# ZYM-PKU/UDiffText

Hardware: AMD Instinct MI355X
Metric: 512x512 50-step denoised images/sec (UDiffText hot path: conditioner + 50 CFG Euler steps + VAE decode) (higher is better)
Workload: dtype bf16; 1 GPU; 512x512, 50 Euler/DDIM(eta 0) steps, CFG 5.0, 9-char labels, noise_iters 0; global batch 4 per step sharded over 1 GPU(s) = 4 images per GPU in micro-batches of 4: every UNet call runs ONE batch of 4 (8 samples with CFG); 3 such batch(es) in flight per GPU on separate launch streams; BASELINE.json configs[1]; global_batch=4, weights=synthetic (name-keyed recipe), 1361.2 M parameters, launch=hipGraph replay of the sampler steps, in_flight=3, batches_per_unet_call=1

## Files before the change

udifftext_amd/csrc/gemm.hip:

```cpp
#include "common.h"
#include <stdio.h>
#include <stdlib.h>
#include <string.h>
#include <atomic>
#include <cmath>

hipError_t udt_lean_launch_gemm(int cfg, const void* lparams, int smem, int G, int geglu, int ln, hipStream_t s);
hipError_t udt_lean_launch_conv3(const void* c3params, hipStream_t s);

namespace {
#include "tile_common.h"

struct GemmParams {
  const uint16_t* a;
  const uint16_t* a2;
  const uint16_t* w;
  const uint16_t* zero;
  const float* bias;
  const uint16_t* res;
  const float* rowvec;
  void* out;
  const float* colscale;
  const float* in_scsh;
  float* colstats;
// ... 821 lines not shown
  t.G = round_workgroups(units);
  int nb = g_n_block.load(std::memory_order_relaxed);
  if (nb <= 0) nb = (t.tiles_m <= 8) ? t.tiles_n : 8;
  if (nb > t.tiles_n) nb = t.tiles_n;
  t.n_block = nb;
  return true;
}

size_t lean_workspace(const LeanPlan& t) {
  return t.splitk > 1 ? G8_HEADER_BYTES + (size_t)t.tiles * t.splitk * t.bm * t.bn * sizeof(float) : 0;
}

std::atomic<int> g_lean_conv{-1};
std::atomic<int> g_wide_conv{-2};
int wide_conv_mode() {
  int v = g_wide_conv.load(std::memory_order_relaxed);
  if (v == -2) {
    const char* e = getenv("UDT_WIDE_CONV");
    v = e ? atoi(e) : -1;
    g_wide_conv.store(v, std::memory_order_relaxed);
  }
  return v;
}
#ifdef UDT_MEASURE
std::atomic<int> g_lconv_dbg{0};
#endif

std::atomic<int> g_wide_lanes_eff{-2};
double wide_lanes_eff() {
  int v = g_wide_lanes_eff.load(std::memory_order_relaxed);
  if (v == -2) {
    const char* e = getenv("UDT_WIDE_LANES_EFF");
    v = e ? atoi(e) : 70;
    g_wide_lanes_eff.store(v, std::memory_order_relaxed);
  }
  return v / 100.0;
}

int conv_chunk_slices(long long tiles, int slots, int chunks, int knob) {
  long long sk = 1;
  if (tiles <= 1023) {
    if (knob > 1) { sk = knob; if (sk > chunks) sk = chunks; }
    else if (knob < 0 && tiles * 2 <= slots && chunks >= 10) { sk = slots / tiles; if (sk > chunks / 4) sk = chunks / 4; }
    if (sk < 1) sk = 1;
  }
  return (int)sk;
}

bool lean_conv_plan(const udt_gemm_desc* d, lg::C3Params& c, bool want_stats) {
  int on = g_lean_conv.load(std::memory_order_relaxed);
  if (on < 0) {
    const char* e = getenv("UDT_LEAN_CONV");
    on = (e && e[0] == '0') ? 0 : 1;
    g_lean_conv.store(on, std::memory_order_relaxed);
  }
  if (!on || lean_mode() == 0) return false;
  if (d->flags != UDT_GEMM_CONV || d->ksize != 3 || d->stride != 1 || d->pad_t != 1 || d->pad_l != 1) return false;
  if (d->C2 != 0 || d->in_scsh || d->colscale || d->batch > 1) return false;
  if (want_stats && !lean_stats_enabled()) return false;
  if (d->N < 128 || d->N % 8 != 0 || d->C1 <= 0 || d->C1 % 64 != 0) return false;
  if (d->upsample != 0 && d->upsample != 1 && d->upsample != 2) return false;
  const bool phase = d->upsample == 2, ups = d->upsample == 1;
  const int nph = phase ? 4 : 1;
  if (d->Hout != (d->Hin << (d->upsample ? 1 : 0)) || d->Wout != (d->Win << (d->upsample ? 1 : 0))) return false;
  if (phase && d->ldw > 0 && d->ldw < 4 * d->C1) return false;
  const int Ht = phase ? d->Hin : d->Hout, Wt = phase ? d->Win : d->Wout;
  c.bn = 128; c.wgm = 2;
  bool wide = false;
  int wide_slots = device_cus();
  {
    const int wm = wide_conv_mode();
    if (wm != 0 && !ups && d->N % 160 == 0 && Wt % 16 == 0 && Ht % 16 == 0) {
      const int cus = device_cus(), share = d->cu_share > 1 ? d->cu_share : 1;
      wide_slots = cus / share > 0 ? cus / share : 1;
      const long long wt = (long long)(d->M / 256) * (d->N / 160);
      const long long sk = conv_chunk_slices(wt, wide_slots, d->C1 / 64, lean_splitk_knob());
      const long long units = wt * sk;
      const long long rounds = (units + cus - 1) / cus;
      const double eff = units > cus ? (double)units / (double)(rounds * cus) : ((double)units * share >= cus ? 1.0 : (double)units * share / cus);
      wide = (wm > 0) || (sk <= 2 && eff >= ((share >= 3 && share_of(d) >= 3) ? wide_lanes_eff() : 0.85));
    }
  }
  if (wide) { c.geo = phase ? 6 : 3; c.tw = 16; c.th = 16; c.bn = 160; c.wgm = 4; }
  else if (Wt % 16 == 0 && Ht % 8 == 0) { c.geo = ups ? 2 : phase ? 4 : 0; c.tw = 16; c.th = 8; }
  else if (!ups && Wt % 8 == 0 && Ht % 8 == 0) { c.geo = phase ? 5 : 1; c.tw = 8; c.th = 8; }
  else return false;
  if (d->ldo % 8 != 0 || (d->residual && d->ldr % 8 != 0)) return false;
  const long long ldw = d->ldw > 0 ? d->ldw : (phase ? 4LL * d->C1 : (long long)d->K);
  if (ldw % 8 != 0) return false;
  c.w_phase = phase ? (d->stride_w > 0 ? d->stride_w : (long long)d->N * ldw) : 0;
  if (phase && (c.w_phase < (long long)d->N * ldw || c.w_phase % 8 != 0)) return false;
  if ((long long)d->M * d->C1 * 2 >= (1LL << 31) || (long long)d->N * ldw * 2 >= (1LL << 31)) return false;
  if ((reinterpret_cast<uintptr_t>(d->out) | reinterpret_cast<uintptr_t>(d->residual) | reinterpret_cast<uintptr_t>(d->bias) |
       reinterpret_cast<uintptr_t>(d->rowvec)) & 15) return false;
  if (d->rowvec && ((d->ld_rowvec > 0 ? d->ld_rowvec : d->N) % 4 != 0)) return false;
  c.dbg = 0;
#ifdef UDT_MEASURE
  c.dbg = g_lconv_dbg.load(std::memory_order_relaxed);
#endif
  c.N = d->N; c.C = d->C1; c.H = d->Hin; c.W = d->Win; c.B = d->M / (d->Hout * d->Wout);
  c.ldw = (int)ldw; c.ldo = d->ldo; c.ldr = d->ldr; c.ldrv = d->ld_rowvec > 0 ? d->ld_rowvec : d->N;
  c.alpha = d->alpha;
  c.tiles_x = Wt / c.tw; c.tiles_y = Ht / c.th;
  c.tiles_m = c.B * c.tiles_x * c.tiles_y;
  c.tiles_n = (d->N + c.bn - 1) / c.bn;
  c.tiles = c.tiles_m * c.tiles_n;
  c.chunks = c.C / 64;
  const int slots = wide ? wide_slots : (2 * device_cus() / share_of(d) > 0 ? 2 * device_cus() / share_of(d) : 1);
  int sk = conv_chunk_slices((long long)c.tiles * nph, slots, c.chunks, lean_splitk_knob());
  while (sk > 1 && (long long)c.tiles * nph * sk * c.tw * c.th * c.bn * 4 > (64LL << 20)) --sk;
  c.ch_per = (c.chunks + sk - 1) / sk;
  c.splitk = (c.chunks + c.ch_per - 1) / c.ch_per;
  c.G = round_workgroups(c.tiles * nph * c.splitk);
  {
    const double patch = (double)((ups ? c.tw / 2 : c.tw) + 2) * ((ups ? c.th / 2 : c.th) + 2) * c.C * 2.0, wtile = (phase ? 4.0 : 9.0) * c.bn * c.C * 2.0;
    int nb = g_n_block.load(std::memory_order_relaxed);
    if (nb <= 0) nb = (int)(std::sqrt(64.0 * patch / wtile) + 0.5);
    if (nb < 1) nb = 1;
    if (nb > c.tiles_n) nb = c.tiles_n;
    c.n_block = nb;
  }
  c.a_bytes = (unsigned)((long long)c.B * d->Hin * d->Win * d->C1 * 2);
  c.w_bytes = (unsigned)((long long)d->N * ldw * 2);
  c.counters = nullptr; c.slabs = nullptr;
  return true;
}

int lean_conv_phases(const lg::C3Params& c) { return c.geo >= 4 ? 4 : 1; }

size_t lean_conv_workspace(const lg::C3Params& c) {
  return c.splitk > 1 ? G8_HEADER_BYTES + (size_t)c.tiles * lean_conv_phases(c) * c.splitk * c.tw * c.th * c.bn * sizeof(float) : 0;
}

bool lean_stats_probe(const udt_gemm_desc* d, int& rows, int& slots) {
  if (d->in_scsh) return false;
  {
    lg::C3Params c3;
    if (lean_conv_plan(d, c3, true)) {
      rows = c3.tw * c3.th / c3.wgm;
      slots = c3.tiles_m * c3.wgm * lean_conv_phases(c3);
      return true;
    }
  }
  if ((d->flags & UDT_GEMM_CONV) && d->ksize == 3) return false;
  LeanPlan lt;
  if (lean_plan(d, lt, true)) {
    rows = lt.stats_rows;
    slots = lt.tiles_m * (lt.bm / lt.stats_rows);
    return true;
  }
  return false;
}
}

extern "C" int udt_debug_set(const char* key, int32_t value) {
  if (!key) return UDT_ERR_BAD_ARG;
  if (!strcmp(key, "n_block")) { g_n_block.store(value); return UDT_OK; }
  if (!strcmp(key, "rows_epi")) { g_rows_epi.store(value ? 1 : 0); return UDT_OK; }
  if (!strcmp(key, "lean")) { g_lean.store(value < 0 ? -2 : value); return UDT_OK; }
  if (!strcmp(key, "rowres")) { g_rowres.store(value < 0 ? 1 : (value ? 1 : 0)); return UDT_OK; }
  if (!strcmp(key, "wide_lanes_eff")) { g_wide_lanes_eff.store(value < 0 ? -2 : value); return UDT_OK; }
  if (!strcmp(key, "conv_n4")) { g_conv_n4.store(value < 0 ? -2 : (value ? 1 : 0)); return UDT_OK; }
  if (!strcmp(key, "lean256_lanes")) { g_lean256_lanes.store(value < 0 ? -2 : (value ? 1 : 0)); return UDT_OK; }
  if (!strcmp(key, "lean_splitk")) { g_lean_splitk.store(value); return UDT_OK; }
  if (!strcmp(key, "share_splitk")) { g_share_splitk.store(value < 0 ? -2 : (value ? 1 : 0)); return UDT_OK; }
  if (!strcmp(key, "lean_conv")) { g_lean_conv.store(value < 0 ? -1 : (value ? 1 : 0)); return UDT_OK; }
  if (!strcmp(key, "wide_conv")) { g_wide_conv.store(value < 0 ? -1 : (value ? 1 : 0)); return UDT_OK; }
#ifdef UDT_MEASURE
  if (!strcmp(key, "lconv_dbg")) { g_lconv_dbg.store(value); return UDT_OK; }
  static const struct { const char* k; int bit; } bits[] = {{"no_xchg", 28}, {"no_epi", 27}, {"no_store", 26}, {"no_res", 25},
                                                            {"no_bias", 24}, {"no_fast", 22}};
  for (const auto& b : bits)
    if (!strcmp(key, b.k)) {
      int cur = g_dbg_bits.load();
      g_dbg_bits.store((cur & ~(1 << b.bit)) | (value ? (1 << b.bit) : 0));
      return UDT_OK;
    }
#endif
  return UDT_ERR_BAD_ARG;
}

extern "C" int udt_check_async_error(void* workspace, size_t workspace_bytes, void* stream) {
  if (!workspace || workspace_bytes < G8_HEADER_BYTES) return UDT_ERR_BAD_ARG;
  hipStream_t s = reinterpret_cast<hipStream_t>(stream);
  int err = 0;
  hipError_t e = hipMemcpyAsync(&err, reinterpret_cast<int*>(workspace) + 1023, sizeof(int), hipMemcpyDeviceToHost, s);
  if (e == hipSuccess) e = hipStreamSynchronize(s);
  if (e != hipSuccess) return udt_set_hip_error(e);
  if (err == 0) return UDT_OK;
  e = hipMemsetAsync(workspace, 0, G8_HEADER_BYTES, s);
// ... 7 lines not shown
extern "C" int32_t udt_gemm_q8_ok(const udt_gemm_desc* d) {
  if (!d || !d->q8_out || d->M <= 0 || d->N <= 0 || d->K <= 0) return 0;
  LeanPlan lt;
  return lean_plan(d, lt, d->colstats != nullptr) ? 1 : 0;
}

extern "C" int32_t udt_gemm_rowstat_parts(const udt_gemm_desc* d) {
  if (!d || d->M <= 0 || d->N <= 0 || d->K <= 0) return 0;
  udt_gemm_desc t = *d;
  alignas(16) static const uint64_t probe_dst[2] = {0, 0};
  if (!t.q8_out) { t.q8_out = const_cast<uint64_t*>(probe_dst); t.q8_scale = const_cast<uint64_t*>(probe_dst); if (t.ld_q8 <= 0) t.ld_q8 = (t.N + 15) / 16 * 16; }
  LeanPlan lt;
  if (!lean_plan(&t, lt, false) || lt.cfg != 1 || (d->flags & UDT_GEMM_GEGLU)) return 0;
  return (d->N + 63) / 64;
}
extern "C" int32_t udt_gemm_in_scsh_ok(const udt_gemm_desc* d) {
  if (!d || d->K <= 0 || d->K % BK != 0) return 0;
  c3p::Geo ge;
  return conv3p_geometry(d, ge, true) ? 1 : 0;
}

extern "C" int32_t udt_gemm_up4_ok(const udt_gemm_desc* d) {
  if (!d || d->upsample != 2) return 0;
  lg::C3Params c3;
  return lean_conv_plan(d, c3, d->colstats != nullptr) ? 1 : 0;
}

extern "C" int udt_gn_silu_conv3x3_fwd(const udt_gemm_desc* d, void* workspace, size_t workspace_bytes, void* stream) {
  if (!d || !(d->flags & UDT_GEMM_CONV) || d->ksize != 3 || d->stride != 1 || d->pad_t != 1 || d->pad_l != 1 || !d->in_scsh)
    return UDT_ERR_BAD_ARG;
  return udt_gemm(d, workspace, workspace_bytes, stream);
}

extern "C" int udt_ln_gemm_fwd(const udt_gemm_desc* d, void* workspace, size_t workspace_bytes, void* stream) {
  if (!d || !d->ln_colsum || !d->bias || !(d->ln_eps > 0.f)) return UDT_ERR_BAD_ARG;
  LeanPlan lt;
  if (!lean_plan(d, lt, false)) return UDT_ERR_BAD_SHAPE;
  return udt_gemm(d, workspace, workspace_bytes, stream);
}

extern "C" size_t udt_gemm_workspace_bytes(const udt_gemm_desc* d) {
  if (!d || d->K <= 0 || d->M <= 0 || d->N <= 0 || d->K % k_tile(d) != 0) return 0;
  if (conv_n4_applies(d)) return 0;
  {
    LeanPlan lt;
    if (lean_plan(d, lt, d->colstats != nullptr)) return lean_workspace(lt);
// ... 162 lines not shown
        udt_prof_tag(profl.rec, tag);
      }
      const bool geglu = (d->flags & UDT_GEMM_GEGLU) != 0, ln = d->ln_colsum != nullptr;
      hipError_t el;
      el = udt_lean_launch_gemm(lt.cfg, &lp, lt.smem, lt.G, geglu ? 1 : 0, ln ? 1 : 0, s);
      if (el != hipSuccess) return udt_set_hip_error(el);
      return UDT_OK;
    }
  }
  if (d->ln_colsum) return UDT_ERR_BAD_ARG;
  {
    lg::C3Params c3;
    if (lean_conv_plan(d, c3, d->colstats != nullptr)) {
      c3.colstats = d->colstats;
      c3.a = p.a; c3.w = p.w; c3.bias = p.bias; c3.res = p.res; c3.rowvec = p.rowvec; c3.out = reinterpret_cast<uint16_t*>(d->out);
      if (c3.splitk > 1) {
        if (!workspace || workspace_bytes < lean_conv_workspace(c3)) return UDT_ERR_WORKSPACE;
        c3.counters = reinterpret_cast<int*>(workspace);
        c3.slabs = reinterpret_cast<float*>(reinterpret_cast<char*>(workspace) + G8_HEADER_BYTES);
      }
      UdtProfScope profc(cls, s);
      if (profc.rec) {
        char tag[96];
        snprintf(tag, sizeof(tag), "%s%s M=%d N=%d K=%d %dx%d tile=%dx%d units=%d splitk=%d nb=%d%s", (c3.geo == 3 || c3.geo == 6) ? "wconv3" : "lconv3",
                 (d->upsample && c3.geo != 6) ? "+up" : "", d->M, d->N, d->K,
                 d->Hin, d->Win, c3.tw, c3.th, c3.tiles * lean_conv_phases(c3) * c3.splitk, c3.splitk, c3.n_block,
                 d->upsample == 2 ? " up4" : "");
        udt_prof_tag(profc.rec, tag);
      }
      const hipError_t ec = udt_lean_launch_conv3(&c3, s);
      if (ec != hipSuccess) return udt_set_hip_error(ec);
      return UDT_OK;
    }
  }
  {
    c3p::CParams cp;
    if (conv3p_geometry(d, cp.geo, d->in_scsh != nullptr)) {
      const TilePlan t3 = plan_tiles3p(d, cp.geo);
      p.tiles_m = t3.tiles_m; p.tiles_n = t3.tiles_n; p.tiles_per_batch = t3.tiles_m * t3.tiles_n;
      {
        const double patch = (double)cp.geo.prows_img * cp.geo.NI * cp.geo.C * 2.0;
        const double wtile = 9.0 * t3.bn * cp.geo.C * 2.0;
        const double S = (double)(t3.tiles < t3.G ? t3.tiles : t3.G) / 8.0;
        int nb = (int)(std::sqrt((S < 1.0 ? 1.0 : S) * patch / wtile) + 0.5);
        if (nb < 1) nb = 1;
        if (nb > t3.tiles_n) nb = t3.tiles_n;
        p.n_block = nb;
      }
      p.n_ktiles = t3.nkt;
      p.total_iters = t3.total;
// ... 110 lines not shown
```

udifftext_amd/csrc/lean.h:

```cpp
#pragma once

namespace lg {

using g8::wait_vm;
UDT_DEVINL void raw_barrier() {
  asm volatile("s_waitcnt lgkmcnt(0)" ::: "memory");
  __builtin_amdgcn_s_barrier();
  asm volatile("" ::: "memory");
}
using g8::buf_lds16;
using g8::OOB;

typedef __attribute__((ext_vector_type(2))) __bf16 bf2_t;
UDT_DEVINL float dot2_bf16(uint32_t a, uint32_t b, float c) {
  return __builtin_amdgcn_fdot2_f32_bf16(__builtin_bit_cast(bf2_t, a), __builtin_bit_cast(bf2_t, b), c, false);
}

template <int CPR, int RPI>
UDT_DEVINL void wave_colstats(char* wl, int lane, const float (&cs)[8], const float (&cq)[8], float* dst, bool col_ok) {
#pragma unroll
  for (int h = 0; h < 2; ++h) {
    f32x4 a = {cs[4 * h + 0], cs[4 * h + 1], cs[4 * h + 2], cs[4 * h + 3]};
    f32x4 b = {cq[4 * h + 0], cq[4 * h + 1], cq[4 * h + 2], cq[4 * h + 3]};
    *reinterpret_cast<f32x4*>(wl + lane * 64 + h * 16) = a;
// ... 563 lines not shown
              cs[2 * j + 1] += bb; cq[2 * j + 1] += bb * bb;
            }
          }
        }
      }
    }
    if constexpr (STATS) {
      const int slot = (m0 + row0) / WROWS;
      wave_colstats<CPR, RPI>(wl, lane, cs, cq, p.colstats + ((long long)slot * p.N + n) * 2, col_ok);
    }
  }
}


template <int MAXN>
UDT_DEVINL void wait_vm_upto(int n) {
  if constexpr (MAXN == 0) wait_vm<0>();
  else {
    if (n >= MAXN) wait_vm<MAXN>();
    else wait_vm_upto<MAXN - 1>(n);
  }
}

template <int TW, int TH, bool UPS>
struct C3Geo {
  static constexpr int PX = TW * TH;
  static constexpr int TM = PX / 64;
  static constexpr int PW = (UPS ? TW / 2 : TW) + 2, PH = (UPS ? TH / 2 : TH) + 2;
  static constexpr int PROWS = PW * PH;
  static constexpr int PIECES = (PROWS + 7) / 8;
  static constexpr int PATCH_BYTES = PIECES * 1024;
  static constexpr int W_BYTES = 128 * ROW_BYTES;
  static constexpr int NRING = (3 * W_BYTES + 2 * PATCH_BYTES <= 80 * 1024) ? 3 : 2;
  static constexpr int RING = NRING * W_BYTES + 2 * PATCH_BYTES;
  static constexpr int STAGING = 4 * TM * 32 * 256;
  static constexpr int SMEM = RING > STAGING ? RING : STAGING;
  static_assert(PX == 128 || PX == 64, "128 or 64 output pixels per workgroup");
  static_assert(SMEM <= 80 * 1024, "two workgroups per CU");
};

template <int TW, int TH, bool UPS, bool STATS = false, bool PHASE = false>
__global__ void __launch_bounds__(256, 2) lconv3_kernel(const C3Params p) {
  static_assert(!(UPS && PHASE), "the phase form runs on the low-resolution geometries");
  using Geo = C3Geo<TW, TH, UPS>;
  constexpr int NT = PHASE ? 4 : 9;
  constexpr int NW = 4, TM = Geo::TM, TN = 2, BN = 128, BMPX = Geo::PX;
  constexpr int C3_PW = Geo::PW, C3_PROWS = Geo::PROWS, C3_PIECES = Geo::PIECES, C3_PATCH_BYTES = Geo::PATCH_BYTES;
  constexpr int C3_W_BYTES = Geo::W_BYTES, C3_TW = TW, C3_TH = TH;
  constexpr int WROWS = TM * 32;
  constexpr int WP = 4;
  constexpr int PP = (C3_PIECES + NW - 1) / NW;
  constexpr int EROW = 64 * 4;
  extern __shared__ __attribute__((aligned(16))) char smem[];
  char* const wring = smem;
  constexpr int NR = Geo::NRING;
  char* const patches = smem + NR * C3_W_BYTES;

  const int tid = threadIdx.x;
  const int wave = __builtin_amdgcn_readfirstlane(tid >> 6);
  const int lane = tid & 63;
  const int l31 = lane & 31;
  const int hi = lane >> 5;
  const int l3 = lane >> 3;
  const int pslot = lane & 7;
  const int wm = wave >> 1, wn = wave & 1;
  const int row0 = wm * WROWS, col0 = wn * 64;
  const int swz_w = (l31 >> 1) & 7;
  const int w_frag_row = (col0 + l31) * ROW_BYTES;

  const int unit = range_index(blockIdx.x, p.G);
  if (unit >= p.tiles * p.splitk * (PHASE ? 4 : 1)) return;
  const int phase = PHASE ? unit / (p.tiles * p.splitk) : 0;
  const int pha = phase >> 1, phb = phase & 1;
  const int ptile = unit / p.splitk;
// ... 11 lines not shown
  }
  const int per_img = p.tiles_x * p.tiles_y;
  const int b = tile_m / per_img;
  const int rt = tile_m - b * per_img;
  const int ty = rt / p.tiles_x;
  const int y0 = ty * C3_TH, x0 = (rt - ty * p.tiles_x) * C3_TW;
  const int c0 = slice * p.ch_per;
  int c1 = c0 + p.ch_per;
  if (c1 > p.chunks) c1 = p.chunks;

  const __amdgpu_buffer_rsrc_t rsrc_a = __builtin_amdgcn_make_buffer_rsrc(const_cast<uint16_t*>(p.a), 0, p.a_bytes, 0x00020000);
  const __amdgpu_buffer_rsrc_t rsrc_w =
      __builtin_amdgcn_make_buffer_rsrc(const_cast<uint16_t*>(p.w) + (PHASE ? (long long)phase * p.w_phase : 0LL), 0, p.w_bytes, 0x00020000);
  auto patch_swz = [](int prow, int yy) { return ((prow - 2 * yy) >> 1) & 7; };
  unsigned w_voff[WP], p_voff[PP];
  int p_piece[PP];
#pragma unroll
  for (int i = 0; i < WP; ++i) {
    const int row = (wave + NW * i) * 8 + l3;
    const int kw = (pslot ^ ((row >> 1) & 7)) * 8;
    const int n = n0 + row;
    w_voff[i] = (n < p.N) ? (unsigned)(((long long)n * p.ldw + kw) * 2) : OOB;
  }
#pragma unroll
  for (int i = 0; i < PP; ++i) {
    int idx = wave + NW * i;
    while (idx >= C3_PIECES) idx -= NW;
    p_piece[i] = idx;
    const int prow = idx * 8 + l3;
    const int yy = prow / C3_PW;
    const int xx = prow - yy * C3_PW;
    const int gy = (UPS ? (y0 >> 1) : y0) + yy - 1, gx = (UPS ? (x0 >> 1) : x0) + xx - 1;
    const bool ok = (prow < C3_PROWS) && ((unsigned)gy < (unsigned)p.H) && ((unsigned)gx < (unsigned)p.W);
    const int koff = (pslot ^ patch_swz(prow, yy)) * 8;
    p_voff[i] = ok ? (unsigned)(((((long long)b * p.H + gy) * p.W + gx) * p.C + koff) * 2) : OOB;
  }
  int a_prow[TM], a_py[TM];
#pragma unroll
  for (int tm = 0; tm < TM; ++tm) {
    const int ml = row0 + tm * 32 + l31;
    const int py = ml / TW, px = ml - py * TW;
    a_py[tm] = PHASE ? py + pha : py;
    a_prow[tm] = UPS ? (py | (px << 16)) : PHASE ? ((py + pha) * C3_PW + px + phb) : (py * C3_PW + px);
  }
  auto issue_w = [&](int st, int c, int tap) {
    const int soff = (tap * p.C + c * 64) * 2;
    char* wbuf = wring + st * C3_W_BYTES;
#pragma unroll
    for (int i = 0; i < WP; ++i) buf_lds16(rsrc_w, wbuf + (wave + NW * i) * 1024, w_voff[i], soff);
  };
  auto issue_patch = [&](int c) {
    char* pbuf = patches + (c & 1) * C3_PATCH_BYTES;
#pragma unroll
    for (int i = 0; i < PP; ++i) buf_lds16(rsrc_a, pbuf + p_piece[i] * 1024, p_voff[i], c * 128);
  };

  f32x16 acc[TM][TN];
#pragma unroll
  for (int i = 0; i < TM; ++i)
#pragma unroll
    for (int j = 0; j < TN; ++j)
#pragma unroll
      for (int r = 0; r < 16; ++r) acc[i][j][r] = 0.f;

  issue_patch(c0);
#pragma unroll
  for (int j = 0; j < NR - 1; ++j) issue_w(j, c0, j);
  static_assert(NR - 1 < NT, "the ring's prologue stays inside the first chunk");
  int st = 0;
  for (int c = c0; c < c1; ++c) {
    const bool nxt = (c + 1 < c1);
    const char* pbuf = patches + (c & 1) * C3_PATCH_BYTES;
#pragma unroll
    for (int tap = 0; tap < NT; ++tap) {
      {
        const int w_ahead = nxt ? NR - 2 : ((NT - 1 - tap) < NR - 2 ? (NT - 1 - tap) : NR - 2);
        const bool patch_ahead = nxt && tap >= 1 && tap <= NR - 1;
        wait_vm_upto<(NR - 2) * WP + PP>(w_ahead * WP + (patch_ahead ? PP : 0));
      }
      raw_barrier();
      if (!UDT_DBG(p.dbg, 0)) {
        const int ahead = tap + NR - 1;
        int s2 = st + NR - 1;
        if (s2 >= NR) s2 -= NR;
        if (ahead < NT) issue_w(s2, c, ahead);
        else if (nxt) issue_w(s2, c + 1, ahead - NT);
      }
      if (tap == 0 && nxt && !UDT_DBG(p.dbg, 1)) issue_patch(c + 1);
      const int dy = PHASE ? tap >> 1 : tap / 3, dx = PHASE ? tap & 1 : tap - dy * 3;
      const char* wbuf = wring + st * C3_W_BYTES;
      bf16x8_t fx[4][TM], fw[4][TN];
      if (!UDT_DBG(p.dbg, 3)) {
#pragma unroll
        for (int t = 0; t < TM; ++t) {
          int prow, yy;
          if constexpr (UPS) {
            const int py = a_prow[t] & 0xffff, px = a_prow[t] >> 16;
            yy = ((py + dy - 1) >> 1) + 1;
            prow = yy * C3_PW + (((px + dx - 1) >> 1) + 1);
          } else {
            yy = a_py[t] + dy;
            prow = a_prow[t] + dy * C3_PW + dx;
          }
          const int arow = prow * ROW_BYTES, aswz = patch_swz(prow, yy);
#pragma unroll
          for (int ks = 0; ks < 4; ++ks) fx[ks][t] = lds_read_frag(pbuf + arow + (((ks * 2 + hi) ^ aswz) << 4));
        }
#pragma unroll
        for (int ks = 0; ks < 4; ++ks) {
          const int slot = ((ks * 2 + hi) ^ swz_w) << 4;
#pragma unroll
          for (int t = 0; t < TN; ++t) fw[ks][t] = lds_read_frag(wbuf + w_frag_row + t * 32 * ROW_BYTES + slot);
        }
      }
      if (UDT_DBG(p.dbg, 2)) {
#pragma unroll
        for (int ks = 0; ks < 4; ++ks) {
#pragma unroll
          for (int tm = 0; tm < TM; ++tm) asm volatile("" ::"v"(fx[ks][tm]));
#pragma unroll
          for (int tn = 0; tn < TN; ++tn) asm volatile("" ::"v"(fw[ks][tn]));
        }
      } else {
#pragma unroll
        for (int ks = 0; ks < 4; ++ks)
#pragma unroll
          for (int tm = 0; tm < TM; ++tm)
// ... 63 lines not shown
      for (int q = 0; q < 4; ++q) {
        const int chunk = (tn * 8 + q * 2 + hi) ^ (row & 7);
        f32x4 v = {acc[tm][tn][q * 4 + 0], acc[tm][tn][q * 4 + 1], acc[tm][tn][q * 4 + 2], acc[tm][tn][q * 4 + 3]};
        *reinterpret_cast<f32x4*>(wl + row * EROW + chunk * 16) = v;
      }
  }
  const int rl = lane >> 3, c8 = lane & 7;
  const int n = n0 + col0 + c8 * 8;
  const bool col_ok = n < p.N;
  f32x4 b0 = {0.f, 0.f, 0.f, 0.f}, b1 = b0;
  if (col_ok) {
    if (p.bias) {
      b0 = *reinterpret_cast<const f32x4*>(p.bias + n);
      b1 = *reinterpret_cast<const f32x4*>(p.bias + n + 4);
    }
    if (p.rowvec) {
      const float* rvp = p.rowvec + (long long)b * p.ldrv + n;
      const f32x4 r0 = *reinterpret_cast<const f32x4*>(rvp), r1 = *reinterpret_cast<const f32x4*>(rvp + 4);
#pragma unroll
      for (int j = 0; j < 4; ++j) b0[j] += r0[j], b1[j] += r1[j];
    }
  }
  constexpr int NIT = TM * 4;
  const int Ho = (UPS || PHASE) ? 2 * p.H : p.H, Wo = (UPS || PHASE) ? 2 * p.W : p.W;
  long long mrow[NIT];
#pragma unroll
  for (int i = 0; i < NIT; ++i) {
    const int ml = row0 + i * 8 + rl;
    const int py = ml / TW, px = ml - py * TW;
    mrow[i] = PHASE ? ((long long)b * Ho + (2 * (y0 + py) + pha)) * Wo + (2 * (x0 + px) + phb)
                    : ((long long)b * Ho + (y0 + py)) * Wo + (x0 + px);
  }
  u32x4 rv[NIT];
  if (p.res) {
#pragma unroll
    for (int i = 0; i < NIT; ++i) {
      u32x4 z = {0u, 0u, 0u, 0u};
      rv[i] = z;
      if (col_ok) rv[i] = *reinterpret_cast<const u32x4*>(p.res + mrow[i] * p.ldr + n);
    }
  }
  float cs[8], cq[8];
#pragma unroll
  for (int j = 0; j < 8; ++j) cs[j] = cq[j] = 0.f;
#pragma unroll
  for (int i = 0; i < NIT; ++i) {
    const int row = i * 8 + rl;
// ... 38 lines not shown
```

udifftext_amd/csrc/lean.hip:

```cpp
#include "common.h"
#include <stdio.h>
#include <stdlib.h>
#include <atomic>

namespace {
#include "tile_common.h"
#include "lean_params.h"
#include "lean.h"
#include "wide.h"
#include "rowres.h"

template <int NW, int WGM, int WGN, int TM, int TN, int NST, int TMB = TM>
hipError_t launch_lean(const lg::LParams& lp, int smem, int G, bool geglu, bool ln, hipStream_t s) {
  static AttrOnce once[5];
  const void* fn;
  const bool stats = lp.colstats != nullptr;
  if constexpr (NW == 4 && NST == 2) {
    if (stats) {
      fn = (const void*)lg::lgemm_kernel<NW, WGM, WGN, TM, TN, NST, false, false, TMB, true>;
      hipError_t e = once[4].ensure(fn, smem);
      if (e != hipSuccess) return e;
      void* args[] = {const_cast<lg::LParams*>(&lp)};
      return hipLaunchKernel(fn, dim3(G), dim3(NW * 64), args, smem, s);
    }
// ... 14 lines not shown
template <bool GEGLU, bool LN, bool STATS, bool FP8, bool EMIT>
hipError_t launch_lean_mx8_k(const lg::LParams& lp, int smem, int G, hipStream_t s) {
  static AttrOnce once;
  const void* fn = (const void*)lg::lgemm_kernel<4, 2, 2, 2, 2, 2, GEGLU, LN, 2, STATS, FP8, EMIT>;
  hipError_t e = once.ensure(fn, smem);
  if (e != hipSuccess) return e;
  void* args[] = {const_cast<lg::LParams*>(&lp)};
  return hipLaunchKernel(fn, dim3(G), dim3(256), args, smem, s);
}
hipError_t launch_lean_mx8(const lg::LParams& lp, int smem, int G, bool geglu, bool ln, bool fp8, bool emit, hipStream_t s) {
  const bool stats = lp.colstats != nullptr;
  if (!fp8) {
    if (emit && !geglu && !ln && !stats) return launch_lean_mx8_k<false, false, false, false, true>(lp, smem, G, s);
    return hipErrorInvalidValue;
  }
  if (geglu) return (ln && emit && !stats) ? launch_lean_mx8_k<true, true, false, true, true>(lp, smem, G, s) : hipErrorInvalidValue;
  if (ln) return stats ? hipErrorInvalidValue
                 : emit ? launch_lean_mx8_k<false, true, false, true, true>(lp, smem, G, s)
                        : launch_lean_mx8_k<false, true, false, true, false>(lp, smem, G, s);
  if (stats) return emit ? hipErrorInvalidValue : launch_lean_mx8_k<false, false, true, true, false>(lp, smem, G, s);
  return emit ? launch_lean_mx8_k<false, false, false, true, true>(lp, smem, G, s) : launch_lean_mx8_k<false, false, false, true, false>(lp, smem, G, s);
}

template <int TW, int TH, bool UPS, bool STATS, bool PHASE>
hipError_t launch_lconv3s(const lg::C3Params& c3, hipStream_t s) {
  static AttrOnce once;
  constexpr int smem = lg::C3Geo<TW, TH, UPS>::SMEM;
  hipError_t e = once.ensure(reinterpret_cast<const void*>(lg::lconv3_kernel<TW, TH, UPS, STATS, PHASE>), smem);
  if (e != hipSuccess) return e;
  hipLaunchKernelGGL((lg::lconv3_kernel<TW, TH, UPS, STATS, PHASE>), dim3(c3.G), dim3(256), smem, s, c3);
  return hipGetLastError();
}
template <int TW, int TH, bool UPS, bool PHASE = false>
hipError_t launch_lconv3(const lg::C3Params& c3, hipStream_t s) {
  return c3.colstats ? launch_lconv3s<TW, TH, UPS, true, PHASE>(c3, s) : launch_lconv3s<TW, TH, UPS, false, PHASE>(c3, s);
}

template <bool STATS, bool PHASE>
hipError_t launch_wconv3s(const lg::C3Params& c3, hipStream_t s) {
  static AttrOnce once;
  constexpr int smem = wd::WGeo::SMEM;
  hipError_t e = once.ensure(reinterpret_cast<const void*>(wd::wconv3_kernel<STATS, PHASE>), smem);
  if (e != hipSuccess) return e;
  hipLaunchKernelGGL((wd::wconv3_kernel<STATS, PHASE>), dim3(c3.G), dim3(256), smem, s, c3);
  return hipGetLastError();
}
template <int KT, bool GEGLU, bool EMIT = false>
hipError_t launch_rowres(const lg::LParams& lp, int G, hipStream_t s) {
  static AttrOnce once;
  constexpr int smem = rr::RGeo<KT, GEGLU>::SMEM;
  hipError_t e = once.ensure(reinterpret_cast<const void*>(rr::rgemm_kernel<KT, GEGLU, EMIT>), smem);
  if (e != hipSuccess) return e;
  hipLaunchKernelGGL((rr::rgemm_kernel<KT, GEGLU, EMIT>), dim3(G), dim3(256), smem, s, lp);
  return hipGetLastError();
}

template <bool PHASE>
hipError_t launch_wconv3(const lg::C3Params& c3, hipStream_t s) {
// ... 2 lines not shown

}

hipError_t udt_lean_launch_gemm(int cfg, const void* lparams, int smem, int G, int geglu, int ln, hipStream_t s) {
  const lg::LParams& lp = *static_cast<const lg::LParams*>(lparams);
  const bool fp8 = lp.a_scale != nullptr, emit = lp.q8_out != nullptr;
  if (cfg == 7 && emit && !fp8 && !geglu && ln && lp.K == 320) return launch_rowres<5, false, true>(lp, G, s);
  if (fp8 || emit) return cfg == 1 ? launch_lean_mx8(lp, smem, G, geglu != 0, ln != 0, fp8, emit, s) : hipErrorInvalidValue;
  switch (cfg) {
    case 1: return launch_lean<4, 2, 2, 2, 2, 2>(lp, smem, G, geglu != 0, ln != 0, s);
    case 6: return launch_lean<8, 2, 4, 4, 2, 2, 1>(lp, smem, G, geglu != 0, ln != 0, s);
    case 5: return geglu ? hipErrorInvalidValue : launch_lean<4, 4, 1, 1, 5, 2>(lp, smem, G, false, ln != 0, s);
    case 7:
      if (!ln || lp.K != 320) return hipErrorInvalidValue;
      return geglu ? launch_rowres<5, true>(lp, G, s) : launch_rowres<5, false>(lp, G, s);
    default: return hipErrorInvalidValue;
  }
}

hipError_t udt_lean_launch_conv3(const void* c3params, hipStream_t s) {
  const lg::C3Params& c3 = *static_cast<const lg::C3Params*>(c3params);
  return c3.geo == 3 ? launch_wconv3<false>(c3, s) : c3.geo == 6 ? launch_wconv3<true>(c3, s) : c3.geo == 2 ? launch_lconv3<16, 8, true>(c3, s)
         : c3.geo == 4 ? launch_lconv3<16, 8, false, true>(c3, s) : c3.geo == 5 ? launch_lconv3<8, 8, false, true>(c3, s)
         : c3.geo == 1 ? launch_lconv3<8, 8, false>(c3, s) : launch_lconv3<16, 8, false>(c3, s);
}
```

udifftext_amd/csrc/lean_params.h:

```cpp
#pragma once

namespace lg {

struct LParams {
  const uint16_t* a;
  const uint16_t* a2;
  const uint16_t* w;
  const float* bias;
  const uint16_t* res;
  const float* rowvec;
  const float* ln_s;
  uint16_t* out;
  int M, N, K;
  int lda, ldw, ldo, ldr, ldrv, rows_per_batch;
  float alpha, ln_eps;
  int tiles_m, tiles_n, n_block, tiles;
  int nkt;
  int splitk, kt_per;
  unsigned a_bytes, w_bytes;
  int kt_split, lda2;
  unsigned a2_bytes;
  int G;
  int* counters;
  float* slabs;
// ... 9 lines not shown
  float q8_fixed_mul;
  float* rowstat_out;
};

struct C3Params {
  const uint16_t* a;
  const uint16_t* w;
  const float* bias;
  const uint16_t* res;
  const float* rowvec;
  uint16_t* out;
  int N, C;
  int B, H, W;
  int ldw, ldo, ldr, ldrv;
  float alpha;
  int tiles_x, tiles_y, tiles_m, tiles_n, n_block, tiles;
  int chunks, splitk, ch_per;
  unsigned a_bytes, w_bytes;
  int G;
  int* counters;
  float* slabs;
  float* colstats;
  int geo, tw, th;
  int bn, wgm;
  long long w_phase;
  int dbg;
};

}
```

Baseline: 10.77 images/s.

## Add stride-2 3x3 conv path to lean implicit-GEMM conv kernel with parity-plane patches

Extends the lean conv3 planner and kernel to handle stride-2 3x3 convolutions (the UNet downsample convs, likely also in the VAE encoder path). The input patch is split into four parity planes, and the taps are reordered so each plane is loaded just in time into a single patch buffer. This replaces the previous fallback GEMM path for these layers. It adds a new geometry (geo 7), heuristics that skip small or CU-saturating shapes, and more complex wait and prefetch scheduling, which carries correctness risk.

```diff
diff --git a/udifftext_amd/csrc/gemm.hip b/udifftext_amd/csrc/gemm.hip
--- a/udifftext_amd/csrc/gemm.hip
+++ b/udifftext_amd/csrc/gemm.hip
@@ -867,6 +867,17 @@
   }
   return v;
 }
+std::atomic<int> g_conv_s2{-2};
+int conv_s2_mode() {
+  int v = g_conv_s2.load(std::memory_order_relaxed);
+  if (v == -2) {
+    const char* e = getenv("UDT_CONV_S2");
+    v = e ? atoi(e) : 1;
+    if (v < 0 || v > 2) v = 1;
+    g_conv_s2.store(v, std::memory_order_relaxed);
+  }
+  return v;
+}
 #ifdef UDT_MEASURE
 std::atomic<int> g_lconv_dbg{0};
 #endif
@@ -900,14 +911,21 @@
     g_lean_conv.store(on, std::memory_order_relaxed);
   }
   if (!on || lean_mode() == 0) return false;
-  if (d->flags != UDT_GEMM_CONV || d->ksize != 3 || d->stride != 1 || d->pad_t != 1 || d->pad_l != 1) return false;
+  if (d->flags != UDT_GEMM_CONV || d->ksize != 3) return false;
+  const bool s2 = d->stride == 2;
+  if (s2) {
+    if (conv_s2_mode() == 0 || d->upsample != 0 || d->pad_t != d->pad_l || (d->pad_t != 0 && d->pad_t != 1)) return false;
+    if (d->Hin != 2 * d->Hout || d->Win != 2 * d->Wout || d->Hout % 8 != 0 || d->Wout % 8 != 0) return false;
+    if (conv_s2_mode() != 2 && d->M < 512) return false;
+    if (conv_s2_mode() != 2 && d->C1 < 256 && (long long)(d->M / 64) * ((d->N + 127) / 128) > 4LL * device_cus()) return false;
+  } else if (d->stride != 1 || d->pad_t != 1 || d->pad_l != 1) return false;
   if (d->C2 != 0 || d->in_scsh || d->colscale || d->batch > 1) return false;
   if (want_stats && !lean_stats_enabled()) return false;
   if (d->N < 128 || d->N % 8 != 0 || d->C1 <= 0 || d->C1 % 64 != 0) return false;
   if (d->upsample != 0 && d->upsample != 1 && d->upsample != 2) return false;
   const bool phase = d->upsample == 2, ups = d->upsample == 1;
   const int nph = phase ? 4 : 1;
-  if (d->Hout != (d->Hin << (d->upsample ? 1 : 0)) || d->Wout != (d->Win << (d->upsample ? 1 : 0))) return false;
+  if (!s2 && (d->Hout != (d->Hin << (d->upsample ? 1 : 0)) || d->Wout != (d->Win << (d->upsample ? 1 : 0)))) return false;
   if (phase && d->ldw > 0 && d->ldw < 4 * d->C1) return false;
   const int Ht = phase ? d->Hin : d->Hout, Wt = phase ? d->Win : d->Wout;
   c.bn = 128; c.wgm = 2;
@@ -915,7 +933,7 @@
   int wide_slots = device_cus();
   {
     const int wm = wide_conv_mode();
-    if (wm != 0 && !ups && d->N % 160 == 0 && Wt % 16 == 0 && Ht % 16 == 0) {
+    if (wm != 0 && !ups && !s2 && d->N % 160 == 0 && Wt % 16 == 0 && Ht % 16 == 0) {
       const int cus = device_cus(), share = d->cu_share > 1 ? d->cu_share : 1;
       wide_slots = cus / share > 0 ? cus / share : 1;
       const long long wt = (long long)(d->M / 256) * (d->N / 160);
@@ -927,6 +945,7 @@
     }
   }
   if (wide) { c.geo = phase ? 6 : 3; c.tw = 16; c.th = 16; c.bn = 160; c.wgm = 4; }
+  else if (s2) { c.geo = 7; c.tw = 8; c.th = 8; }
   else if (Wt % 16 == 0 && Ht % 8 == 0) { c.geo = ups ? 2 : phase ? 4 : 0; c.tw = 16; c.th = 8; }
   else if (!ups && Wt % 8 == 0 && Ht % 8 == 0) { c.geo = phase ? 5 : 1; c.tw = 8; c.th = 8; }
   else return false;
@@ -935,7 +954,7 @@
   if (ldw % 8 != 0) return false;
   c.w_phase = phase ? (d->stride_w > 0 ? d->stride_w : (long long)d->N * ldw) : 0;
   if (phase && (c.w_phase < (long long)d->N * ldw || c.w_phase % 8 != 0)) return false;
-  if ((long long)d->M * d->C1 * 2 >= (1LL << 31) || (long long)d->N * ldw * 2 >= (1LL << 31)) return false;
+  if ((long long)d->M * (s2 ? 4 : 1) * d->C1 * 2 >= (1LL << 31) || (long long)d->N * ldw * 2 >= (1LL << 31)) return false;
   if ((reinterpret_cast<uintptr_t>(d->out) | reinterpret_cast<uintptr_t>(d->residual) | reinterpret_cast<uintptr_t>(d->bias) |
        reinterpret_cast<uintptr_t>(d->rowvec)) & 15) return false;
   if (d->rowvec && ((d->ld_rowvec > 0 ? d->ld_rowvec : d->N) % 4 != 0)) return false;
@@ -945,7 +964,7 @@
 #endif
   c.N = d->N; c.C = d->C1; c.H = d->Hin; c.W = d->Win; c.B = d->M / (d->Hout * d->Wout);
   c.ldw = (int)ldw; c.ldo = d->ldo; c.ldr = d->ldr; c.ldrv = d->ld_rowvec > 0 ? d->ld_rowvec : d->N;
-  c.alpha = d->alpha;
+  c.alpha = d->alpha; c.pad = d->pad_t;
   c.tiles_x = Wt / c.tw; c.tiles_y = Ht / c.th;
   c.tiles_m = c.B * c.tiles_x * c.tiles_y;
   c.tiles_n = (d->N + c.bn - 1) / c.bn;
@@ -958,7 +977,7 @@
   c.splitk = (c.chunks + c.ch_per - 1) / c.ch_per;
   c.G = round_workgroups(c.tiles * nph * c.splitk);
   {
-    const double patch = (double)((ups ? c.tw / 2 : c.tw) + 2) * ((ups ? c.th / 2 : c.th) + 2) * c.C * 2.0, wtile = (phase ? 4.0 : 9.0) * c.bn * c.C * 2.0;
+    const double patch = (s2 ? (double)(2 * c.tw + 1) * (2 * c.th + 1) : (double)((ups ? c.tw / 2 : c.tw) + 2) * ((ups ? c.th / 2 : c.th) + 2)) * c.C * 2.0, wtile = (phase ? 4.0 : 9.0) * c.bn * c.C * 2.0;
     int nb = g_n_block.load(std::memory_order_relaxed);
     if (nb <= 0) nb = (int)(std::sqrt(64.0 * patch / wtile) + 0.5);
     if (nb < 1) nb = 1;
@@ -971,7 +990,7 @@
   return true;
 }
 
-int lean_conv_phases(const lg::C3Params& c) { return c.geo >= 4 ? 4 : 1; }
+int lean_conv_phases(const lg::C3Params& c) { return (c.geo >= 4 && c.geo <= 6) ? 4 : 1; }
 
 size_t lean_conv_workspace(const lg::C3Params& c) {
   return c.splitk > 1 ? G8_HEADER_BYTES + (size_t)c.tiles * lean_conv_phases(c) * c.splitk * c.tw * c.th * c.bn * sizeof(float) : 0;
@@ -1011,6 +1030,7 @@
   if (!strcmp(key, "share_splitk")) { g_share_splitk.store(value < 0 ? -2 : (value ? 1 : 0)); return UDT_OK; }
   if (!strcmp(key, "lean_conv")) { g_lean_conv.store(value < 0 ? -1 : (value ? 1 : 0)); return UDT_OK; }
   if (!strcmp(key, "wide_conv")) { g_wide_conv.store(value < 0 ? -1 : (value ? 1 : 0)); return UDT_OK; }
+  if (!strcmp(key, "conv_s2")) { g_conv_s2.store((value < 0 || value > 2) ? -2 : value); return UDT_OK; }
 #ifdef UDT_MEASURE
   if (!strcmp(key, "lconv_dbg")) { g_lconv_dbg.store(value); return UDT_OK; }
   static const struct { const char* k; int bit; } bits[] = {{"no_xchg", 28}, {"no_epi", 27}, {"no_store", 26}, {"no_res", 25},
@@ -1064,6 +1084,12 @@
 
 extern "C" int32_t udt_gemm_up4_ok(const udt_gemm_desc* d) {
   if (!d || d->upsample != 2) return 0;
+  lg::C3Params c3;
+  return lean_conv_plan(d, c3, d->colstats != nullptr) ? 1 : 0;
+}
+
+extern "C" int32_t udt_gemm_stride2_ok(const udt_gemm_desc* d) {
+  if (!d || d->stride != 2) return 0;
   lg::C3Params c3;
   return lean_conv_plan(d, c3, d->colstats != nullptr) ? 1 : 0;
 }
@@ -1272,10 +1298,10 @@
       UdtProfScope profc(cls, s);
       if (profc.rec) {
         char tag[96];
-        snprintf(tag, sizeof(tag), "%s%s M=%d N=%d K=%d %dx%d tile=%dx%d units=%d splitk=%d nb=%d%s", (c3.geo == 3 || c3.geo == 6) ? "wconv3" : "lconv3",
+        snprintf(tag, sizeof(tag), "%s%s M=%d N=%d K=%d %dx%d tile=%dx%d units=%d splitk=%d nb=%d%s%s", (c3.geo == 3 || c3.geo == 6) ? "wconv3" : "lconv3",
                  (d->upsample && c3.geo != 6) ? "+up" : "", d->M, d->N, d->K,
                  d->Hin, d->Win, c3.tw, c3.th, c3.tiles * lean_conv_phases(c3) * c3.splitk, c3.splitk, c3.n_block,
-                 d->upsample == 2 ? " up4" : "");
+                 d->upsample == 2 ? " up4" : "", c3.geo == 7 ? " s2" : "");
         udt_prof_tag(profc.rec, tag);
       }
       const hipError_t ec = udt_lean_launch_conv3(&c3, s);
diff --git a/udifftext_amd/csrc/lean.h b/udifftext_amd/csrc/lean.h
--- a/udifftext_amd/csrc/lean.h
+++ b/udifftext_amd/csrc/lean.h
@@ -609,34 +609,49 @@
   }
 }
 
-template <int TW, int TH, bool UPS>
+template <int TW, int TH>
+struct S2Planes {
+  static constexpr int pw(int q) { return TW + ((q & 1) ? 0 : 1); }
+  static constexpr int ph(int q) { return TH + ((q & 2) ? 0 : 1); }
+  static constexpr int rows(int q) { return pw(q) * ph(q); }
+  static constexpr int pieces(int q) { return (rows(q) + 7) / 8; }
+  static constexpr int base(int q) { return q == 0 ? 0 : base(q - 1) + pieces(q - 1); }
+  static constexpr int instr(int q) { return (pieces(q) + 3) / 4; }
+  static constexpr int ibase(int q) { return q == 0 ? 0 : ibase(q - 1) + instr(q - 1); }
+};
+UDT_DEVINL constexpr int s2_ord(int i) { return i == 0 ? 0 : i == 1 ? 2 : i == 2 ? 6 : i == 3 ? 8 : i == 4 ? 1 : i == 5 ? 7 : i == 6 ? 3 : i == 7 ? 5 : 4; }
+
+template <int TW, int TH, bool UPS, bool S2 = false>
 struct C3Geo {
   static constexpr int PX = TW * TH;
   static constexpr int TM = PX / 64;
   static constexpr int PW = (UPS ? TW / 2 : TW) + 2, PH = (UPS ? TH / 2 : TH) + 2;
   static constexpr int PROWS = PW * PH;
-  static constexpr int PIECES = (PROWS + 7) / 8;
+  static constexpr int PIECES = S2 ? S2Planes<TW, TH>::base(4) : (PROWS + 7) / 8;
   static constexpr int PATCH_BYTES = PIECES * 1024;
+  static constexpr int NPATCH = S2 ? 1 : 2;
   static constexpr int W_BYTES = 128 * ROW_BYTES;
-  static constexpr int NRING = (3 * W_BYTES + 2 * PATCH_BYTES <= 80 * 1024) ? 3 : 2;
-  static constexpr int RING = NRING * W_BYTES + 2 * PATCH_BYTES;
+  static constexpr int NRING = (3 * W_BYTES + NPATCH * PATCH_BYTES <= 80 * 1024) ? 3 : 2;
+  static constexpr int RING = NRING * W_BYTES + NPATCH * PATCH_BYTES;
   static constexpr int STAGING = 4 * TM * 32 * 256;
   static constexpr int SMEM = RING > STAGING ? RING : STAGING;
   static_assert(PX == 128 || PX == 64, "128 or 64 output pixels per workgroup");
   static_assert(SMEM <= 80 * 1024, "two workgroups per CU");
 };
 
-template <int TW, int TH, bool UPS, bool STATS = false, bool PHASE = false>
+template <int TW, int TH, bool UPS, bool STATS = false, bool PHASE = false, bool S2 = false>
 __global__ void __launch_bounds__(256, 2) lconv3_kernel(const C3Params p) {
   static_assert(!(UPS && PHASE), "the phase form runs on the low-resolution geometries");
-  using Geo = C3Geo<TW, TH, UPS>;
+  static_assert(!S2 || (!UPS && !PHASE && TW == 8 && TH == 8), "the stride-2 form: 8 x 8 output tiles (S2Planes)");
+  using Geo = C3Geo<TW, TH, UPS, S2>;
+  using Pl = S2Planes<TW, TH>;
   constexpr int NT = PHASE ? 4 : 9;
   constexpr int NW = 4, TM = Geo::TM, TN = 2, BN = 128, BMPX = Geo::PX;
   constexpr int C3_PW = Geo::PW, C3_PROWS = Geo::PROWS, C3_PIECES = Geo::PIECES, C3_PATCH_BYTES = Geo::PATCH_BYTES;
   constexpr int C3_W_BYTES = Geo::W_BYTES, C3_TW = TW, C3_TH = TH;
   constexpr int WROWS = TM * 32;
   constexpr int WP = 4;
-  constexpr int PP = (C3_PIECES + NW - 1) / NW;
+  constexpr int PP = S2 ? Pl::ibase(4) : (C3_PIECES + NW - 1) / NW;
   constexpr int EROW = 64 * 4;
   extern __shared__ __attribute__((aligned(16))) char smem[];
   char* const wring = smem;
@@ -694,18 +709,38 @@
     const int n = n0 + row;
     w_voff[i] = (n < p.N) ? (unsigned)(((long long)n * p.ldw + kw) * 2) : OOB;
   }
-#pragma unroll
-  for (int i = 0; i < PP; ++i) {
-    int idx = wave + NW * i;
-    while (idx >= C3_PIECES) idx -= NW;
-    p_piece[i] = idx;
-    const int prow = idx * 8 + l3;
-    const int yy = prow / C3_PW;
-    const int xx = prow - yy * C3_PW;
-    const int gy = (UPS ? (y0 >> 1) : y0) + yy - 1, gx = (UPS ? (x0 >> 1) : x0) + xx - 1;
-    const bool ok = (prow < C3_PROWS) && ((unsigned)gy < (unsigned)p.H) && ((unsigned)gx < (unsigned)p.W);
-    const int koff = (pslot ^ patch_swz(prow, yy)) * 8;
-    p_voff[i] = ok ? (unsigned)(((((long long)b * p.H + gy) * p.W + gx) * p.C + koff) * 2) : OOB;
+  auto s2_swz = [](int yy, int xx) { return ((yy * TW + xx) >> 1) & 7; };
+  if constexpr (S2) {
+#pragma unroll
+    for (int q = 0; q < 4; ++q) {
+#pragma unroll
+      for (int i = 0; i < Pl::instr(q); ++i) {
+        int idx = wave + NW * i;
+        while (idx >= Pl::pieces(q)) idx -= NW;
+        p_piece[Pl::ibase(q) + i] = Pl::base(q) + idx;
+        const int r = idx * 8 + l3;
+        const int yy = r / Pl::pw(q);
+        const int xx = r - yy * Pl::pw(q);
+        const int gy = 2 * (y0 + yy) + (q >> 1) - p.pad, gx = 2 * (x0 + xx) + (q & 1) - p.pad;
+        const bool ok = (r < Pl::rows(q)) && ((unsigned)gy < (unsigned)p.H) && ((unsigned)gx < (unsigned)p.W);
+        const int koff = (pslot ^ s2_swz(yy, xx)) * 8;
+        p_voff[Pl::ibase(q) + i] = ok ? (unsigned)(((((long long)b * p.H + gy) * p.W + gx) * p.C + koff) * 2) : OOB;
+      }
+    }
+  } else {
+#pragma unroll
+    for (int i = 0; i < PP; ++i) {
+      int idx = wave + NW * i;
+      while (idx >= C3_PIECES) idx -= NW;
+      p_piece[i] = idx;
+      const int prow = idx * 8 + l3;
+      const int yy = prow / C3_PW;
+      const int xx = prow - yy * C3_PW;
+      const int gy = (UPS ? (y0 >> 1) : y0) + yy - 1, gx = (UPS ? (x0 >> 1) : x0) + xx - 1;
+      const bool ok = (prow < C3_PROWS) && ((unsigned)gy < (unsigned)p.H) && ((unsigned)gx < (unsigned)p.W);
+      const int koff = (pslot ^ patch_swz(prow, yy)) * 8;
+      p_voff[i] = ok ? (unsigned)(((((long long)b * p.H + gy) * p.W + gx) * p.C + koff) * 2) : OOB;
+    }
   }
   int a_prow[TM], a_py[TM];
 #pragma unroll
@@ -713,7 +748,7 @@
     const int ml = row0 + tm * 32 + l31;
     const int py = ml / TW, px = ml - py * TW;
     a_py[tm] = PHASE ? py + pha : py;
-    a_prow[tm] = UPS ? (py | (px << 16)) : PHASE ? ((py + pha) * C3_PW + px + phb) : (py * C3_PW + px);
+    a_prow[tm] = (UPS || S2) ? (py | (px << 16)) : PHASE ? ((py + pha) * C3_PW + px + phb) : (py * C3_PW + px);
   }
   auto issue_w = [&](int st, int c, int tap) {
     const int soff = (tap * p.C + c * 64) * 2;
@@ -722,10 +757,15 @@
     for (int i = 0; i < WP; ++i) buf_lds16(rsrc_w, wbuf + (wave + NW * i) * 1024, w_voff[i], soff);
   };
   auto issue_patch = [&](int c) {
-    char* pbuf = patches + (c & 1) * C3_PATCH_BYTES;
+    char* pbuf = patches + (S2 ? 0 : (c & 1) * C3_PATCH_BYTES);
 #pragma unroll
     for (int i = 0; i < PP; ++i) buf_lds16(rsrc_a, pbuf + p_piece[i] * 1024, p_voff[i], c * 128);
   };
+  auto issue_plane = [&](int q, int c) {
+#pragma unroll
+    for (int i = 0; i < PP; ++i)
+      if (i >= Pl::ibase(q) && i < Pl::ibase(q) + Pl::instr(q)) buf_lds16(rsrc_a, patches + p_piece[i] * 1024, p_voff[i], c * 128);
+  };
 
   f32x16 acc[TM][TN];
 #pragma unroll
@@ -737,15 +777,20 @@
 
   issue_patch(c0);
 #pragma unroll
-  for (int j = 0; j < NR - 1; ++j) issue_w(j, c0, j);
+  for (int j = 0; j < NR - 1; ++j) issue_w(j, c0, S2 ? s2_ord(j) : j);
   static_assert(NR - 1 < NT, "the ring's prologue stays inside the first chunk");
+  static_assert(!S2 || NR == 2, "the stride-2 form's waits are written for the two-stage ring");
   int st = 0;
   for (int c = c0; c < c1; ++c) {
     const bool nxt = (c + 1 < c1);
-    const char* pbuf = patches + (c & 1) * C3_PATCH_BYTES;
+    const char* pbuf = patches + (S2 ? 0 : (c & 1) * C3_PATCH_BYTES);
 #pragma unroll
     for (int tap = 0; tap < NT; ++tap) {
-      {
+      if constexpr (S2) {
+        const int keep = tap == 0 ? (c > c0 ? Pl::instr(2) : 0) : tap == 1 ? (c > c0 ? Pl::instr(3) : 0)
+                         : tap == 5 ? (nxt ? Pl::instr(0) : 0) : tap == 7 ? (nxt ? Pl::instr(1) : 0) : 0;
+        wait_vm_upto<Pl::instr(0)>(keep);
+      } else {
         const int w_ahead = nxt ? NR - 2 : ((NT - 1 - tap) < NR - 2 ? (NT - 1 - tap) : NR - 2);
         const bool patch_ahead = nxt && tap >= 1 && tap <= NR - 1;
         wait_vm_upto<(NR - 2) * WP + PP>(w_ahead * WP + (patch_ahead ? PP : 0));
@@ -755,26 +800,44 @@
         const int ahead = tap + NR - 1;
         int s2 = st + NR - 1;
         if (s2 >= NR) s2 -= NR;
-        if (ahead < NT) issue_w(s2, c, ahead);
-        else if (nxt) issue_w(s2, c + 1, ahead - NT);
-      }
-      if (tap == 0 && nxt && !UDT_DBG(p.dbg, 1)) issue_patch(c + 1);
-      const int dy = PHASE ? tap >> 1 : tap / 3, dx = PHASE ? tap & 1 : tap - dy * 3;
+        if (ahead < NT) issue_w(s2, c, S2 ? s2_ord(ahead) : ahead);
+        else if (nxt) issue_w(s2, c + 1, S2 ? s2_ord(ahead - NT) : ahead - NT);
+      }
+      if constexpr (S2) {
+        if (!UDT_DBG(p.dbg, 1)) {
+          if (tap == 0 && c > c0) issue_plane(3, c);
+          if (tap == 4 && nxt) issue_plane(0, c + 1);
+          if (tap == 6 && nxt) issue_plane(1, c + 1);
+          if (tap == 8 && nxt) issue_plane(2, c + 1);
+        }
+      } else {
+        if (tap == 0 && nxt && !UDT_DBG(p.dbg, 1)) issue_patch(c + 1);
+      }
+      const int tap9 = S2 ? s2_ord(tap) : tap;
+      const int dy = PHASE ? tap >> 1 : tap9 / 3, dx = PHASE ? tap & 1 : tap9 - dy * 3;
       const char* wbuf = wring + st * C3_W_BYTES;
       bf16x8_t fx[4][TM], fw[4][TN];
       if (!UDT_DBG(p.dbg, 3)) {
 #pragma unroll
         for (int t = 0; t < TM; ++t) {
-          int prow, yy;
-          if constexpr (UPS) {
+          int prow, yy, aswz;
+          if constexpr (S2) {
+            const int q = 2 * (dy & 1) + (dx & 1);
+            const int py = a_prow[t] & 0xffff, px = a_prow[t] >> 16;
+            yy = py + (dy >> 1);
+            prow = Pl::base(q) * 8 + yy * Pl::pw(q) + px + (dx >> 1);
+            aswz = s2_swz(yy, px + (dx >> 1));
+          } else if constexpr (UPS) {
             const int py = a_prow[t] & 0xffff, px = a_prow[t] >> 16;
             yy = ((py + dy - 1) >> 1) + 1;
             prow = yy * C3_PW + (((px + dx - 1) >> 1) + 1);
+            aswz = patch_swz(prow, yy);
           } else {
             yy = a_py[t] + dy;
             prow = a_prow[t] + dy * C3_PW + dx;
-          }
-          const int arow = prow * ROW_BYTES, aswz = patch_swz(prow, yy);
+            aswz = patch_swz(prow, yy);
+          }
+          const int arow = prow * ROW_BYTES;
 #pragma unroll
           for (int ks = 0; ks < 4; ++ks) fx[ks][t] = lds_read_frag(pbuf + arow + (((ks * 2 + hi) ^ aswz) << 4));
         }
@@ -884,7 +947,7 @@
     }
   }
   constexpr int NIT = TM * 4;
-  const int Ho = (UPS || PHASE) ? 2 * p.H : p.H, Wo = (UPS || PHASE) ? 2 * p.W : p.W;
+  const int Ho = S2 ? p.tiles_y * TH : (UPS || PHASE) ? 2 * p.H : p.H, Wo = S2 ? p.tiles_x * TW : (UPS || PHASE) ? 2 * p.W : p.W;
   long long mrow[NIT];
 #pragma unroll
   for (int i = 0; i < NIT; ++i) {
diff --git a/udifftext_amd/csrc/lean.hip b/udifftext_amd/csrc/lean.hip
--- a/udifftext_amd/csrc/lean.hip
+++ b/udifftext_amd/csrc/lean.hip
@@ -60,18 +60,18 @@
   return emit ? launch_lean_mx8_k<false, false, false, true, true>(lp, smem, G, s) : launch_lean_mx8_k<false, false, false, true, false>(lp, smem, G, s);
 }
 
-template <int TW, int TH, bool UPS, bool STATS, bool PHASE>
+template <int TW, int TH, bool UPS, bool STATS, bool PHASE, bool S2>
 hipError_t launch_lconv3s(const lg::C3Params& c3, hipStream_t s) {
   static AttrOnce once;
-  constexpr int smem = lg::C3Geo<TW, TH, UPS>::SMEM;
-  hipError_t e = once.ensure(reinterpret_cast<const void*>(lg::lconv3_kernel<TW, TH, UPS, STATS, PHASE>), smem);
+  constexpr int smem = lg::C3Geo<TW, TH, UPS, S2>::SMEM;
+  hipError_t e = once.ensure(reinterpret_cast<const void*>(lg::lconv3_kernel<TW, TH, UPS, STATS, PHASE, S2>), smem);
   if (e != hipSuccess) return e;
-  hipLaunchKernelGGL((lg::lconv3_kernel<TW, TH, UPS, STATS, PHASE>), dim3(c3.G), dim3(256), smem, s, c3);
+  hipLaunchKernelGGL((lg::lconv3_kernel<TW, TH, UPS, STATS, PHASE, S2>), dim3(c3.G), dim3(256), smem, s, c3);
   return hipGetLastError();
 }
-template <int TW, int TH, bool UPS, bool PHASE = false>
+template <int TW, int TH, bool UPS, bool PHASE = false, bool S2 = false>
 hipError_t launch_lconv3(const lg::C3Params& c3, hipStream_t s) {
-  return c3.colstats ? launch_lconv3s<TW, TH, UPS, true, PHASE>(c3, s) : launch_lconv3s<TW, TH, UPS, false, PHASE>(c3, s);
+  return c3.colstats ? launch_lconv3s<TW, TH, UPS, true, PHASE, S2>(c3, s) : launch_lconv3s<TW, TH, UPS, false, PHASE, S2>(c3, s);
 }
 
 template <bool STATS, bool PHASE>
@@ -120,5 +120,6 @@
   const lg::C3Params& c3 = *static_cast<const lg::C3Params*>(c3params);
   return c3.geo == 3 ? launch_wconv3<false>(c3, s) : c3.geo == 6 ? launch_wconv3<true>(c3, s) : c3.geo == 2 ? launch_lconv3<16, 8, true>(c3, s)
          : c3.geo == 4 ? launch_lconv3<16, 8, false, true>(c3, s) : c3.geo == 5 ? launch_lconv3<8, 8, false, true>(c3, s)
+         : c3.geo == 7 ? launch_lconv3<8, 8, false, false, true>(c3, s)
          : c3.geo == 1 ? launch_lconv3<8, 8, false>(c3, s) : launch_lconv3<16, 8, false>(c3, s);
 }
diff --git a/udifftext_amd/csrc/lean_params.h b/udifftext_amd/csrc/lean_params.h
--- a/udifftext_amd/csrc/lean_params.h
+++ b/udifftext_amd/csrc/lean_params.h
@@ -55,6 +55,7 @@
   float* slabs;
   float* colstats;
   int geo, tw, th;
+  int pad;
   int bn, wgm;
   long long w_phase;
   int dbg;
```

Result: no change. 10.74 images/s (-0.3%).
